# qyber-black/Code-RobChar

Hardware: AMD Instinct MI355X
Metric: MC fidelity evals/sec (N=7, 100 ctrls x 10k draws) (higher is better)
Workload: dtype f64

## Files before the change

### code-robchar_amd/csrc/k_fidelity_chain.inc.h

```cpp
constexpr int kWavesSmall = 5;
constexpr int fid_min_waves(int n, int mode) {
    if (mode == rc::kWeightsAdjugate)
        return n >= 17 ? 1
               : rc::kSumRuleMoments >= 3 ? (n <= 6 ? kWavesSmall : (n <= 7 ? 4 : (n <= 8 ? 3 : (n >= 13 ? 1 : 2))))
                                          : (n <= 6 ? kWavesSmall : (n <= 8 ? 4 : (n == 13 ? 1 : 2)));
    if (mode == rc::kWeightsRows) return n <= 8 ? kWavesSmall : (n <= 12 ? 3 : 2);
    return n <= 6 ? kWavesSmall : (n <= 8 ? 4 : (n <= 10 ? 3 : (n <= 14 ? 2 : 1)));
}
constexpr int fid_phases(int n, int mode) { return n <= 2 ? 1 : (n <= 8 ? 2 : 4); }

#include "philox_core.inc.h"

__device__ unsigned long long g_general_tiles = 0;
__device__ unsigned long long g_polish_tiles[64] = {0};

struct LdsVec {
    double* base;
    int stride;
    __device__ __forceinline__ double& operator[](int i) const { return base[i * stride]; }
};

template <int N, int MODE>
__global__ __launch_bounds__(64, fid_min_waves(N, MODE)) void mc_fid_chain_kernel(const FidParams p) {
    constexpr int G = 3 * N;
    constexpr int PH = fid_phases(N, MODE);
    constexpr int SP = 64 / PH;
    constexpr int kPhaseBytes = SP * G * 8;
    __shared__ __attribute__((aligned(16))) double stage[SP * G];
    __shared__ __attribute__((aligned(16))) double sctab[128];

    const int lane = threadIdx.x;
    const long long tile = blockIdx.x;
    const double2 ent = reinterpret_cast<const double2*>(g_sincos_table)[lane];
    reinterpret_cast<double2*>(sctab)[lane] = ent;
    __builtin_amdgcn_s_setprio(3);
#ifdef RC_STAMPS
    const long long t_begin = __builtin_amdgcn_s_memtime();
    const long long r_begin = __builtin_amdgcn_s_memrealtime();
#endif
    const long long c = tile / p.tiles_per_ctrl;
    const long long kb = (tile - c * p.tiles_per_ctrl) * 64;
    const int nk = (int)((p.K - kb < 64) ? (p.K - kb) : 64);

    const double* xg = p.ctrl + c * (N + 1);
    double x[N + 1];
    bool pad = false;
#pragma unroll
    for (int i = 0; i <= N; ++i) {
        x[i] = xg[i];
        pad |= (x[i] != x[i]);
    }
#ifdef RC_STAMPS
    long long t_ph[4] = {0, 0, 0, 0};
    asm volatile("s_waitcnt lgkmcnt(0)" ::: "memory");
    const long long t_ctrl = __builtin_amdgcn_s_memtime();
#endif
    double* dst = p.fid + c * p.K + kb;
    if (pad) {
        if (lane < nk) dst[lane] = __builtin_nan("");
        return;
    }

    const char* src = (const char*)(p.draws + c * p.draw_cstride + kb * G);
    double gl[G];
#pragma unroll
    for (int ph = 0; ph < PH; ++ph) {
        const int first = ph * SP;
        if (first < nk) {
            const int cnt = (nk - first < SP) ? (nk - first) : SP;
            const int bytes = cnt * G * 8;
            const char* ps = src + (long long)first * G * 8;
            if (p.align16 && !(cnt & 1)) {
#pragma unroll
                for (int it = 0; it < (kPhaseBytes + 1023) / 1024; ++it) {
                    const int off = it * 1024 + lane * 16;
                    if (off < bytes)
                        __builtin_amdgcn_global_load_lds((rc_gptr_t)(ps + off),
                                                         (rc_lptr_t)((char*)stage + it * 1024), 16, 0, rckp::kDrawLoadAux);
                }
            } else {
#pragma unroll 2
                for (int it = 0; it < (kPhaseBytes + 255) / 256; ++it) {
                    const int off = it * 256 + lane * 4;
                    if (off < bytes)
                        __builtin_amdgcn_global_load_lds((rc_gptr_t)(ps + off),
                                                         (rc_lptr_t)((char*)stage + it * 256), 4, 0, rckp::kDrawLoadAux);
                }
            }
            asm volatile("s_waitcnt vmcnt(0)" ::: "memory");
#ifdef RC_STAMPS
            if (ph < 2) t_ph[2 * ph] = __builtin_amdgcn_s_memtime();
#endif
            int rel = lane - first;
            asm volatile("" : "+v"(rel));
            if (rel >= 0 && rel < cnt) {
#pragma unroll
                for (int i = 0; i < G; ++i) gl[i] = stage[rel * G + i];
            }
            asm volatile("s_waitcnt lgkmcnt(0)" ::: "memory");
#ifdef RC_STAMPS
            if (ph < 2) t_ph[2 * ph + 1] = __builtin_amdgcn_s_memtime();
#endif
        }
    }
    __builtin_amdgcn_s_setprio(0);
    __syncthreads();
#ifdef RC_STAMPS
    const long long t_loaded = __builtin_amdgcn_s_memtime();
#endif

    double f = 0.0;
    bool ok = true;
#ifdef RC_STAMPS
    long long t_in[2] = {0, 0};
    if (lane < nk)
        ok = rc::chain_fidelity_fast<N, MODE>(x, p.h0.diag, p.h0.off, [&gl](int i) { return gl[i]; }, p.in, p.out, sctab, f, t_in);
#else
    int extra = 0;
    if (lane < nk)
        ok = rc::chain_fidelity_fast<N, MODE>(x, p.h0.diag, p.h0.off, [&gl](int i) { return gl[i]; }, p.in, p.out, sctab, f,
                                              nullptr, &extra);
    if (extra && lane == 0) atomicAdd(&g_polish_tiles[blockIdx.x & 63u], 1ull);
#endif
    constexpr bool kRepairInRegisters = MODE != rc::kWeightsRows && N <= RC_MAX_NSPIN_FAST;
    unsigned long long badmask = __ballot(lane < nk && !ok);
    if (badmask != 0ull) {
        if (lane == 0) atomicAdd(&g_general_tiles, 1ull);
        if (kRepairInRegisters) {
            const bool bad = (badmask >> lane) & 1ull;
            bool ok2 = true;
            if (bad) {
                const double* gsrc = (const double*)src + (long long)lane * G;
                double f2;
                ok2 = rc::chain_fidelity_fast<N, rc::kWeightsRows>(xg, p.h0.diag, p.h0.off, [gsrc](int i) { return gsrc[i]; },
                                                                   p.in, p.out, sctab, f2);
                if (ok2) f = f2;
            }
            badmask = __ballot(bad && !ok2);
        }
    }
    if (badmask != 0ull) {
        constexpr int CH = (SP * G) / (4 * N);
        const bool bad = (badmask >> lane) & 1ull;
        const int rank = __popcll(badmask & ((1ull << lane) - 1ull));
        const int nbad = __popcll(badmask);
#pragma unroll 1
        for (int c0 = 0; c0 < nbad; c0 += CH) {
            const int rel = rank - c0;
            if (bad && rel >= 0 && rel < CH) {
                const LdsVec vd{stage + rel, CH}, ve{stage + N * CH + rel, CH}, va{stage + 2 * N * CH + rel, CH},
                    vb{stage + 3 * N * CH + rel, CH};
                f = rc::chain_fidelity_general(N, xg, p.h0.diag, p.h0.off,
                                               (const double*)src + (long long)lane * G, p.in, p.out, vd, ve, va, vb);
            }
        }
    }
    if (lane < nk) {
        if (p.nt_store) {
            __attribute__((address_space(1))) double* nt_dst = (__attribute__((address_space(1))) double*)(dst + lane);
            asm volatile("" : "+v"(nt_dst));
            __builtin_nontemporal_store(f, nt_dst);
        } else {
            dst[lane] = f;
        }
    }

#ifdef RC_STAMPS
    __builtin_amdgcn_s_waitcnt(0);
    const long long t_end = __builtin_amdgcn_s_memtime();
    if (lane == 0 && p.stamps) {
        long long* rec = p.stamps + tile * rckp::kStampSlots;
        rec[0] = t_begin;
        rec[1] = t_loaded;
        rec[2] = t_end;
        rec[3] = __builtin_amdgcn_s_memrealtime() - r_begin;
        rec[4] = t_ctrl;
        rec[5] = t_ph[0];
        rec[6] = t_in[0];
        rec[7] = t_in[1];
        rec[8] = (long long)__builtin_amdgcn_s_getreg(4 | (0 << 6) | (31 << 11));
        rec[9] = (long long)__builtin_amdgcn_s_getreg(20 | (0 << 6) | (31 << 11));
        rec[10] = r_begin;
        rec[11] = r_begin + rec[3];
    }
#endif
}

constexpr int kRingMaxN = 16;
constexpr int ring_min_waves(int n) { return n <= 4 ? 5 : (n <= 5 ? 4 : (n <= 6 ? 3 : (n <= 8 ? 2 : 1))); }


template <int N>
__device__ __forceinline__ void ring_tile_fp64(const FidParams& p, const double corner, const long long tile, double* stage,
                                               const double* sctab) {
    constexpr int G = 3 * N;
    constexpr int PH = fid_phases(N, rc::kWeightsRows);
    constexpr int SP = 64 / PH;
    const int lane = threadIdx.x;
    __builtin_amdgcn_s_setprio(3);
    const long long c = tile / p.tiles_per_ctrl;
    const long long kb = (tile - c * p.tiles_per_ctrl) * 64;
    const int nk = (int)((p.K - kb < 64) ? (p.K - kb) : 64);
    const double* xg = p.ctrl + c * (N + 1);
    double x[N + 1];
    bool pad = false;
#pragma unroll
    for (int i = 0; i <= N; ++i) {
        x[i] = xg[i];
        pad |= (x[i] != x[i]);
    }
    double* dst = p.fid + c * p.K + kb;
    if (pad) {
        if (lane < nk) dst[lane] = __builtin_nan("");
        __builtin_amdgcn_s_setprio(0);
        return;
    }
    const char* src = (const char*)(p.draws + c * p.draw_cstride + kb * G);
    double gl[G];
    stage_tile_draws<G, PH>(src, nk, lane, p.align16, stage, gl);
    __builtin_amdgcn_s_setprio(0);

    double f = 0.0;
    bool ok = true;
    if (lane < nk)
        ok = rc::ring_fidelity_fast<N>(x, p.h0.diag, p.h0.off, corner, [&gl](int i) { return gl[i]; }, p.in, p.out, sctab, f);
    const unsigned long long badmask = __ballot(lane < nk && !ok);
    if (badmask) {
        if (lane == 0) atomicAdd(&g_general_tiles, 1ull);
        constexpr int CH = (SP * G) / (6 * N);
        const bool bad = (badmask >> lane) & 1ull;
        const int rank = __popcll(badmask & ((1ull << lane) - 1ull));
        const int nbad = __popcll(badmask);
#pragma unroll 1
        for (int c0 = 0; c0 < nbad; c0 += CH) {
            const int rel = rank - c0;
            if (bad && rel >= 0 && rel < CH) {
                const LdsVec vd{stage + rel, CH}, ve{stage + N * CH + rel, CH};
                LdsVec vz[4] = {{stage + 2 * N * CH + rel, CH}, {stage + 3 * N * CH + rel, CH}, {stage + 4 * N * CH + rel, CH},
                                {stage + 5 * N * CH + rel, CH}};
                const double* gsrc = (const double*)src + (long long)lane * G;
                f = rc::ring_fidelity_general<N>(x, p.h0.diag, p.h0.off, corner, [gsrc](int i) { return gsrc[i]; }, p.in, p.out,
                                                 vd, ve, vz);
            }
        }
    }
    if (lane < nk) dst[lane] = f;
}

template <int N>
__global__ __launch_bounds__(64, ring_min_waves(N)) void mc_fid_ring_kernel(const FidParams p, const double corner) {
    constexpr int G = 3 * N;
    constexpr int SP = 64 / fid_phases(N, rc::kWeightsRows);
    __shared__ __attribute__((aligned(16))) double stage[SP * G];
    __shared__ __attribute__((aligned(16))) double sctab[128];
    const double2 ent = reinterpret_cast<const double2*>(g_sincos_table)[threadIdx.x];
    reinterpret_cast<double2*>(sctab)[threadIdx.x] = ent;
    __syncthreads();
    ring_tile_fp64<N>(p, corner, blockIdx.x, stage, sctab);
}

constexpr int ring_mixed_min_waves(int n) {
    return n <= 4 ? 5 : (n <= 6 ? 4 : (n <= 8 ? 3 : (n == 9 ? (rc::kSumRuleMoments >= 3 ? 2 : 3) : (n <= 13 ? 2 : 1))));
}


template <int N>
__global__ __launch_bounds__(64, ring_mixed_min_waves(N)) void mc_fid_ring_mixed_kernel(const FidParams p, const double corner,
                                                                                        const RingRepairList rl) {
    constexpr int G = 3 * N;
    constexpr int PH = (N == 16) ? 8 : fid_phases(N, rc::kWeightsEnds);
    constexpr int SP = 64 / PH;
    __shared__ __attribute__((aligned(16))) double stage[SP * G];
    __shared__ __attribute__((aligned(16))) double sctab[128];
    const int lane = threadIdx.x;
    const long long tile = blockIdx.x;
    if (blockIdx.x == 0 && lane == 0) *rl.clear = 0ull;
    const double2 ent = reinterpret_cast<const double2*>(g_sincos_table)[lane];
    reinterpret_cast<double2*>(sctab)[lane] = ent;
    __builtin_amdgcn_s_setprio(3);
    const long long c = tile / p.tiles_per_ctrl;
    const long long kb = (tile - c * p.tiles_per_ctrl) * 64;
    const int nk = (int)((p.K - kb < 64) ? (p.K - kb) : 64);
    const double* xg = p.ctrl + c * (N + 1);
    double x[N + 1];
    bool pad = false;
#pragma unroll
    for (int i = 0; i <= N; ++i) {
        x[i] = xg[i];
        pad |= (x[i] != x[i]);
    }
    double* dst = p.fid + c * p.K + kb;
    if (pad) {
        if (lane < nk) dst[lane] = __builtin_nan("");
        return;
    }
    const char* src = (const char*)(p.draws + c * p.draw_cstride + kb * G);
    double gl[G];
    stage_tile_draws<G, PH>(src, nk, lane, p.align16, stage, gl);
    __builtin_amdgcn_s_setprio(0);
    __syncthreads();
    double f = 0.0;
    bool ok = true;
    int extra = 0;
    if (lane < nk)
        ok = rc::ring_fidelity_mixed<N>(x, p.h0.diag, p.h0.off, corner, [&gl](int i) { return gl[i]; }, p.in, p.out, sctab, f,
                                        &extra);
    if (extra && lane == 0) atomicAdd(&g_polish_tiles[blockIdx.x & 63u], 1ull);
    const bool bad = lane < nk && !ok;
    const unsigned long long badmask = __ballot(bad);
    if (badmask) {
        const int first = __ffsll((long long)badmask) - 1;
        unsigned long long base = 0;
        if (lane == first) base = atomicAdd(rl.count, (unsigned long long)__popcll(badmask));
        base = __shfl(base, first, 64);
        if (bad) {
            rl.samples[base + __popcll(badmask & ((1ull << lane) - 1ull))] = c * p.K + kb + lane;
            f = __builtin_nan("");
        }
    }
    if (lane < nk) dst[lane] = f;
}

template <int N>
__global__ __launch_bounds__(64, 1) void mc_fid_ring_repair_kernel(const FidParams p, const double corner, const RingRepairList rl) {
    constexpr int G = 3 * N;
    __shared__ __attribute__((aligned(16))) double work[6 * N * 64];
    __shared__ __attribute__((aligned(16))) double sctab[128];
    const int lane = threadIdx.x;
    const double2 ent = reinterpret_cast<const double2*>(g_sincos_table)[lane];
    reinterpret_cast<double2*>(sctab)[lane] = ent;
// ... 62 lines not shown
```

### code-robchar_amd/csrc/robchar_hip.hip

```cpp
#include <hip/hip_runtime.h>

#include <dlfcn.h>
#include <math.h>
#include <stdint.h>
#include <stdlib.h>
#include <string.h>
#include <atomic>
#include <initializer_list>
#include <mutex>
#include <unordered_map>
#include <thread>
#include <string>
#include <vector>

#include "../../include/robchar_hip.h"
#include "kernel_params.h"
#include "tridiag_core.h"
#include "hermitian_core.h"
#include "csym_core.h"
#include "sort_core.h"
#include "select_core.h"
#include "bootstrap_core.h"
#include "wasserstein_core.h"
#include "lbfgs_core.h"
// ... 57 lines not shown
std::mutex g_cfg_mu;
int g_default_kernel = RC_KERNEL_AUTO;
long long* g_stamps = nullptr;

constexpr int kMaxDevices = 64;
enum { kAttrExpm = 0, kAttrAnyN, kAttrSortMerge, kAttrSortChunk, kAttrMtJump, kAttrMtJumpWide, kAttrCount };
struct RingBuf {
    char* mem = nullptr;
    long long cap = 0;
    int turn = 0;
    unsigned long long last_use = 0;
};
constexpr size_t kMaxRingBufs = 16;
struct DeviceCtx {
    std::mutex mu;
    hipStream_t stream = nullptr;
    void* ws = nullptr;
    size_t ws_bytes = 0;
    std::mutex ring_mu;
    std::unordered_map<hipStream_t, RingBuf> ring_bufs;
    unsigned long long ring_clock = 0;
    std::atomic<bool> attr[kAttrCount];
    DeviceCtx() {
        for (auto& a : attr) a.store(false);
    }
};
DeviceCtx g_ctx[kMaxDevices];

int device_in_range(int device) {
    int n = 0;
    RC_HIP_CHECK(hipGetDeviceCount(&n));
    if (device < 0 || device >= n || device >= kMaxDevices) return fail(RC_EINVAL, "device index out of range");
    return RC_OK;
}

int get_ctx(int device, DeviceCtx** out) {
    if (int rc = device_in_range(device)) return rc;
    RC_HIP_CHECK(hipSetDevice(device));
    if (!g_ctx[device].stream) RC_HIP_CHECK(hipStreamCreateWithFlags(&g_ctx[device].stream, hipStreamNonBlocking));
    *out = &g_ctx[device];
    return RC_OK;
}

int ensure_func_attr(int which, const void* func, int bytes) {
    int dev = 0;
    RC_HIP_CHECK(hipGetDevice(&dev));
    if (dev < 0 || dev >= kMaxDevices) return fail(RC_EINVAL, "device index out of range");
    if (g_ctx[dev].attr[which].load(std::memory_order_acquire)) return RC_OK;
    RC_HIP_CHECK(hipFuncSetAttribute(func, hipFuncAttributeMaxDynamicSharedMemorySize, bytes));
    g_ctx[dev].attr[which].store(true, std::memory_order_release);
    return RC_OK;
}

int ensure_ws(DeviceCtx* ctx, size_t bytes) {
    if (ctx->ws_bytes >= bytes) return RC_OK;
    if (ctx->ws) RC_HIP_CHECK(hipFree(ctx->ws));
    ctx->ws = nullptr;
    ctx->ws_bytes = 0;
    RC_HIP_CHECK(hipMalloc(&ctx->ws, bytes));
    ctx->ws_bytes = bytes;
    return RC_OK;
}

bool is_device_ptr(const void* p) {
    hipPointerAttribute_t attr;
    hipError_t e = hipPointerGetAttributes(&attr, p);
    if (e != hipSuccess) {
        (void)hipGetLastError();
        return false;
    }
    return attr.type == hipMemoryTypeDevice;
}

struct Staging {
    DeviceCtx* ctx = nullptr;
    rcws::Plan plan;
    int in(const void* p, size_t bytes) { return plan.in(p, bytes, is_device_ptr(p)); }
    int out(void* p, size_t bytes, bool always = false) { return plan.out(p, bytes, p && !always && is_device_ptr(p), always); }
    double* ptr(int slot) const { return (double*)plan.ptr(slot, ctx->ws); }
    int stage_in() {
        if (int rc = ensure_ws(ctx, plan.total)) return rc;
        for (int i = 0; i < plan.n; ++i)
            if (const rcws::Slot& s = plan.s[i]; s.input && s.staged)
                RC_HIP_CHECK(hipMemcpyAsync(ptr(i), s.user, s.bytes, hipMemcpyHostToDevice, ctx->stream));
        return RC_OK;
    }
    int stage_out() {
        for (int i = 0; i < plan.n; ++i)
            if (const rcws::Slot& s = plan.s[i]; !s.input && s.staged && s.user)
                RC_HIP_CHECK(hipMemcpyAsync((void*)s.user, ptr(i), s.bytes, s.always ? hipMemcpyDefault : hipMemcpyDeviceToHost,
                                            ctx->stream));
        RC_HIP_CHECK(hipStreamSynchronize(ctx->stream));
        return RC_OK;
    }
};

struct StreamFree {
    void* p;
    hipStream_t s;
    ~StreamFree() {
        if (p) (void)hipFreeAsync(p, s);
    }
};

void fill_h0(StaticH& h0, int N, const double* h0_diag, const double* h0_offdiag) {
    for (int i = 0; i < RC_MAX_NSPIN; ++i) {
        h0.diag[i] = (h0_diag && i < N) ? h0_diag[i] : 0.0;
        h0.off[i] = (i < N - 1) ? (h0_offdiag ? h0_offdiag[i] : 1.0) : 0.0;
    }
}

int check_common(int N, int in, int out, long long C, long long K) {
    if (N < 2 || N > RC_MAX_NSPIN) return fail(RC_EINVAL, "N must be in [2, 32]");
    if (in < 0 || in >= N || out < 0 || out >= N) return fail(RC_EINVAL, "in/out spin index out of range");
    if (C < 0 || K < 0) return fail(RC_EINVAL, "C and K must be non-negative");
    return RC_OK;
}

int ring_buf_reserve(RingBuf& rb, hipStream_t s, long long samples) {
    if (rb.cap >= samples && rb.mem) return RC_OK;
    if (rb.mem) RC_HIP_CHECK(hipFreeAsync(rb.mem, s));
    rb.mem = nullptr;
    rb.cap = 0;
    const long long cap = samples + (samples >> 2);
    RC_HIP_CHECK(hipMallocAsync((void**)&rb.mem, 256 + (size_t)cap * sizeof(long long), s));
    RC_HIP_CHECK(hipMemsetAsync(rb.mem, 0, 256, s));
    rb.cap = cap;
    rb.turn = 0;
    return RC_OK;
}

RingBuf& ring_buf_for(DeviceCtx& ctx, hipStream_t s) {
    auto it = ctx.ring_bufs.find(s);
    if (it == ctx.ring_bufs.end()) {
        if (ctx.ring_bufs.size() >= kMaxRingBufs) {
            auto old = ctx.ring_bufs.begin();
            for (auto j = ctx.ring_bufs.begin(); j != ctx.ring_bufs.end(); ++j)
                if (j->second.last_use < old->second.last_use) old = j;
            if (old->second.mem) (void)hipFree(old->second.mem);
            ctx.ring_bufs.erase(old);
        }
        it = ctx.ring_bufs.emplace(s, RingBuf{}).first;
    }
    it->second.last_use = ++ctx.ring_clock;
    return it->second;
}

constexpr long long kNtStoreTiles = 32768;
std::atomic<long long> g_nt_store_tiles{kNtStoreTiles};

template <int N, int MODE>
int launch_chain(hipStream_t s, const FidParams& p0, long long nt_store_tiles) {
    const long long blocks = p0.ntiles;
    if (blocks > 0x7fffffffLL) return fail(RC_EINVAL, "too many tiles for one launch");
    FidParams p = p0;
    p.nt_store = (blocks < nt_store_tiles) ? 1 : 0;
    hipLaunchKernelGGL((mc_fid_chain_kernel<N, MODE>), dim3((unsigned)blocks), dim3(64), 0, s, p);
    RC_HIP_CHECK(hipGetLastError());
    return RC_OK;
}

int enqueue_expm(hipStream_t s, int N, int in, int out, const double* h0_diag, const double* h0_offdiag, int ring,
                 const double* ctrl, const double* draws, long long draw_cstride, const double* diag_imag,
                 long long imag_cstride, long long C, long long K, double* fid, bool fast_complex_diagonal = false) {
    if (N > RC_MAX_NSPIN_FAST) return fail(RC_EINVAL, "the dense kernels (ring topology, expm) support N <= 16");
    ExpmParams p{};
    p.ctrl = ctrl;
    p.draws = draws;
    p.diag_imag = diag_imag;
    p.fid = fid;
    p.C = C;
    p.K = K;
    p.draw_cstride = draw_cstride;
    p.imag_cstride = imag_cstride;
    p.N = N;
    p.in = in;
    p.out = out;
    p.ring = ring ? 1 : 0;
    fill_h0(p.h0, N, h0_diag, h0_offdiag);
    const size_t lds = (size_t)kExpmWaves * kExpmBufs * N * N * sizeof(cplx);
    if (int rc = ensure_func_attr(kAttrExpm, (const void*)mc_fid_expm_kernel,
                                  kExpmWaves * kExpmBufs * RC_MAX_NSPIN_FAST * RC_MAX_NSPIN_FAST * (int)sizeof(cplx)))
        return rc;
    const long long total = C * K;
    long long blocks = (total + kExpmWaves - 1) / kExpmWaves;
    if (blocks > 256LL * 16) blocks = 256LL * 16;
    if (fast_complex_diagonal && !ring && N <= kCsymMaxN) {
        const long long cblocks = (total + 63) / 64;
        if (cblocks > 0x7fffffffLL) return fail(RC_EINVAL, "too many samples for one launch");
        switch (N) {
#define RC_CSYM_CASE(n) \
    case n: hipLaunchKernelGGL(mc_fid_csym_kernel<n>, dim3((unsigned)cblocks), dim3(64), 0, s, p); break;
            RC_CSYM_CASE(2) RC_CSYM_CASE(3) RC_CSYM_CASE(4) RC_CSYM_CASE(5) RC_CSYM_CASE(6) RC_CSYM_CASE(7) RC_CSYM_CASE(8)
            RC_CSYM_CASE(9) RC_CSYM_CASE(10) RC_CSYM_CASE(11) RC_CSYM_CASE(12)
#undef RC_CSYM_CASE
        }
        p.only_marked = 1;
    }
    hipLaunchKernelGGL(mc_fid_expm_kernel, dim3((unsigned)blocks), dim3(64 * kExpmWaves), lds, s, p);
    RC_HIP_CHECK(hipGetLastError());
    return RC_OK;
}

int draws_align16(const double* draws, long long draw_cstride) {
    return (((uintptr_t)draws & 15) == 0 && (((size_t)draw_cstride * 8) & 15) == 0) ? 1 : 0;
}
size_t draws_bytes(long long C, long long K, int N, long long stride) {
    return (stride == 0 ? (size_t)K * N * 3 : ((size_t)(C - 1) * stride + (size_t)K * N * 3)) * sizeof(double);
}

int enqueue_fidelity(hipStream_t s, int kernel, int N, int in, int out, const double* h0_diag,
                     const double* h0_offdiag, int ring, const double* ctrl, const double* draws,
                     long long draw_cstride, long long C, long long K, double* fid) {
    if (draw_cstride < 0) draw_cstride = K * N * 3;
    if (draw_cstride != 0 && draw_cstride < K * N * 3) return fail(RC_EINVAL, "draws_ctrl_stride overlaps controllers");
    if (int rc = check_common(N, in, out, C, K)) return rc;
    if (C == 0 || K == 0) return RC_OK;
    if (!ctrl || !draws || !fid) return fail(RC_EINVAL, "NULL array pointer");
    const bool ends = (in == 0 && out == N - 1) || (in == N - 1 && out == 0);
    if (ring && N == 2) ring = 0;
    const bool mixed_ring = (kernel == RC_KERNEL_AUTO) && ring && N <= kRingMaxN;
    if (kernel == RC_KERNEL_AUTO)
        kernel = ring ? (N <= kRingMaxN ? RC_KERNEL_RING_HH : RC_KERNEL_JACOBI) : RC_KERNEL_TRIDIAG_ADJ;
    if (kernel == RC_KERNEL_RING_HH) {
        if (!ring) return fail(RC_EINVAL, "RC_KERNEL_RING_HH is the ring-topology kernel (chains: the tridiagonal kernels)");
        if (N > kRingMaxN) return fail(RC_EINVAL, "the lane-per-sample ring kernels support N <= 16");
        FidParams p{};
        p.ctrl = ctrl;
        p.draws = draws;
        p.fid = fid;
        p.C = C;
        p.K = K;
        p.draw_cstride = draw_cstride;
        p.tiles_per_ctrl = (K + 63) / 64;
        p.ntiles = C * p.tiles_per_ctrl;
        p.in = in;
        p.out = out;
        p.align16 = draws_align16(draws, draw_cstride);
        fill_h0(p.h0, N, h0_diag, h0_offdiag);
        if (p.ntiles > 0x7fffffffLL) return fail(RC_EINVAL, "too many tiles for one launch");
        const dim3 grid((unsigned)p.ntiles);
        if (mixed_ring) {
            RingRepairList rl{};
            {
                int dev = 0;
                RC_HIP_CHECK(hipGetDevice(&dev));
                if (dev < 0 || dev >= kMaxDevices) return fail(RC_EINVAL, "device index out of range");
                std::lock_guard<std::mutex> lk(g_ctx[dev].ring_mu);
                RingBuf& rb = ring_buf_for(g_ctx[dev], s);
                if (int rc = ring_buf_reserve(rb, s, C * K)) return rc;
                rl.count = (unsigned long long*)(rb.mem + 64 * rb.turn);
                rl.clear = (unsigned long long*)(rb.mem + 64 * (rb.turn ^ 1));
                rl.samples = (long long*)(rb.mem + 256);
                rb.turn ^= 1;
            }
            static const long long kRepairGrid = [] {
                const char* e = getenv("RC_RING_REPAIR_GRID");
                const long long v = e ? atoll(e) : 0;
                return v > 0 ? v : 1024LL;
            }();
            const long long nwaves = (C * K + 63) / 64;
            const dim3 rgrid((unsigned)(nwaves < kRepairGrid ? nwaves : kRepairGrid));
            if (N > 10) {
                RC_HIP_CHECK((hipError_t)rc_large_ring_launch(N, 1, (void*)s, &p, 1.0, &rl, grid.x, rgrid.x));
                return RC_OK;
            }
            switch (N) {
#define RC_RING_CASE(n)                                                                         \
    case n:                                                                                     \
        hipLaunchKernelGGL(mc_fid_ring_mixed_kernel<n>, grid, dim3(64), 0, s, p, 1.0, rl);      \
        hipLaunchKernelGGL(mc_fid_ring_repair_kernel<n>, rgrid, dim3(64), 0, s, p, 1.0, rl);    \
        break;
                RC_RING_CASE(3) RC_RING_CASE(4) RC_RING_CASE(5) RC_RING_CASE(6) RC_RING_CASE(7) RC_RING_CASE(8) RC_RING_CASE(9)
                RC_RING_CASE(10)
#undef RC_RING_CASE
            }
            RC_HIP_CHECK(hipGetLastError());
            return RC_OK;
        }
        if (N > 10) {
            RC_HIP_CHECK((hipError_t)rc_large_ring_launch(N, 0, (void*)s, &p, 1.0, nullptr, grid.x, 0u));
            return RC_OK;
        }
        switch (N) {
#define RC_RING_CASE(n) \
    case n: hipLaunchKernelGGL(mc_fid_ring_kernel<n>, grid, dim3(64), 0, s, p, 1.0); break;
            RC_RING_CASE(3) RC_RING_CASE(4) RC_RING_CASE(5) RC_RING_CASE(6) RC_RING_CASE(7) RC_RING_CASE(8) RC_RING_CASE(9)
            RC_RING_CASE(10)
#undef RC_RING_CASE
        }
        RC_HIP_CHECK(hipGetLastError());
        return RC_OK;
    }
    if (kernel == RC_KERNEL_TRIDIAG_QL || kernel == RC_KERNEL_TRIDIAG_ADJ) {
        const int mode = (kernel == RC_KERNEL_TRIDIAG_QL) ? rc::kWeightsRows
                                                          : ((ends && N <= 14) ? rc::kWeightsEnds : rc::kWeightsAdjugate);
        if (ring) return fail(RC_EINVAL, "the tridiagonal QL kernel handles chain topology only");
        FidParams p{};
        p.ctrl = ctrl;
        p.draws = draws;
        p.fid = fid;
        p.C = C;
        p.K = K;
        p.draw_cstride = draw_cstride;
        p.tiles_per_ctrl = (K + 63) / 64;
        p.ntiles = C * p.tiles_per_ctrl;
        p.in = in;
        p.out = out;
        p.align16 = draws_align16(draws, draw_cstride);
        p.stamps = g_stamps;
        fill_h0(p.h0, N, h0_diag, h0_offdiag);
        if (N > RC_MAX_NSPIN_CHAIN || (N > RC_MAX_NSPIN_FAST && mode == rc::kWeightsRows)) {
            const long long blocks = p.ntiles;
            if (blocks > 0x7fffffffLL) return fail(RC_EINVAL, "too many tiles for one launch");
            const size_t lds = (size_t)4 * N * 64 * sizeof(double);
            if (int rc = ensure_func_attr(kAttrAnyN, (const void*)mc_fid_chain_anyn_kernel, 4 * RC_MAX_NSPIN * 64 * (int)sizeof(double)))
                return rc;
            hipLaunchKernelGGL(mc_fid_chain_anyn_kernel, dim3((unsigned)blocks), dim3(64), lds, s, p, N);
            RC_HIP_CHECK(hipGetLastError());
            return RC_OK;
        }
        if (N > RC_MAX_NSPIN_FAST) {
            if (p.ntiles > 0x7fffffffLL) return fail(RC_EINVAL, "too many tiles for one launch");
            RC_HIP_CHECK((hipError_t)rc_large_chain_launch(N, (void*)s, &p));
            return RC_OK;
        }
        const long long nt_tiles = g_nt_store_tiles.load(std::memory_order_relaxed);
        switch (N) {
#define RC_CASE(n)                                                                        \
    case n:                                                                               \
        return mode == rc::kWeightsRows ? launch_chain<n, rc::kWeightsRows>(s, p, nt_tiles)         \
               : (mode == rc::kWeightsEnds ? launch_chain<n, rc::kWeightsEnds>(s, p, nt_tiles)      \
                                           : launch_chain<n, rc::kWeightsAdjugate>(s, p, nt_tiles));
#define RC_CASE_ADJ_ROWS(n)                                                               \
    case n:                                                                               \
        return mode == rc::kWeightsRows ? launch_chain<n, rc::kWeightsRows>(s, p, nt_tiles) : launch_chain<n, rc::kWeightsAdjugate>(s, p, nt_tiles);
#ifdef RC_DEV_FEW_N
            RC_CASE(5) RC_CASE(7) RC_CASE(10)
#else
            RC_CASE(2) RC_CASE(3) RC_CASE(4) RC_CASE(5) RC_CASE(6) RC_CASE(7) RC_CASE(8) RC_CASE(9)
            RC_CASE(10) RC_CASE(11) RC_CASE(12) RC_CASE(13) RC_CASE(14) RC_CASE_ADJ_ROWS(15) RC_CASE_ADJ_ROWS(16)
#endif
#undef RC_CASE
#undef RC_CASE_ADJ_ROWS
        }
        return fail(RC_EINVAL, "unsupported N");
    }
    if (N > RC_MAX_NSPIN_FAST) return fail(RC_EINVAL, "the dense kernels (ring topology, expm) support N <= 16");
    if (kernel == RC_KERNEL_EXPM)
        return enqueue_expm(s, N, in, out, h0_diag, h0_offdiag, ring, ctrl, draws, draw_cstride, nullptr, 0, C, K, fid);
    if (kernel == RC_KERNEL_JACOBI) {
        JacParams p{};
        p.ctrl = ctrl;
        p.draws = draws;
        p.fid = fid;
        p.C = C;
        p.K = K;
        p.draw_cstride = draw_cstride;
        p.N = N;
        p.in = in;
        p.out = out;
        p.ring = ring ? 1 : 0;
        fill_h0(p.h0, N, h0_diag, h0_offdiag);
        const long long total = C * K;
        const int spw = (N <= 8) ? 8 : 4;
        long long blocks = (total + kJacWaves * spw - 1) / (kJacWaves * spw);
        if (blocks > 256LL * 16) blocks = 256LL * 16;
        if (N <= 8)
            hipLaunchKernelGGL((mc_fid_jacobi_kernel<8, 8>), dim3((unsigned)blocks), dim3(64 * kJacWaves), 0, s, p);
        else
            hipLaunchKernelGGL((mc_fid_jacobi_kernel<16, 16>), dim3((unsigned)blocks), dim3(64 * kJacWaves), 0, s, p);
        RC_HIP_CHECK(hipGetLastError());
        return RC_OK;
    }
    return fail(RC_EINVAL, "unknown kernel id");
}

int enqueue_reduce(hipStream_t s, const double* fid, long long C, long long K, const double* thr, int nq,
                   double eps, double* rim1, double* stdv, double* minf, double* q, double* sorted_out, bool standalone = false) {
    if (C < 0 || K < 0) return fail(RC_EINVAL, "C and K must be non-negative");
    if (nq < 0 || nq > kMaxQ) return fail(RC_EINVAL, "nq must be in [0, 8]");
    if (nq > 0 && !thr) return fail(RC_EINVAL, "q_thresholds is NULL");
    if (C == 0) return RC_OK;
    if (K == 0) return fail(RC_EINVAL, "K must be positive for a reduction");
    if (!fid) return fail(RC_EINVAL, "NULL fid pointer");
    if (C > 0x7fffffffLL) return fail(RC_EINVAL, "too many controllers for one launch");
    RedParams p{};
    p.fid = fid;
    p.C = C;
    p.K = K;
    p.nq = nq;
    for (int j = 0; j < nq; ++j) p.thr[j] = thr[j];
    p.eps = eps;
    p.rim1 = rim1;
    p.stdv = stdv;
    p.minf = minf;
    p.q = q;
    if (rim1 || stdv || minf || q) {
        if (K <= kWaveRowMaxK && C >= 64) {
            const dim3 grid((unsigned)((C + 3) / 4));
            if (nq == 0)
                hipLaunchKernelGGL(reduce_rows_wave_kernel<0>, grid, dim3(256), 0, s, p);
            else if (nq <= 2)
                hipLaunchKernelGGL(reduce_rows_wave_kernel<2>, grid, dim3(256), 0, s, p);
            else
                hipLaunchKernelGGL(reduce_rows_wave_kernel<kMaxQ>, grid, dim3(256), 0, s, p);
        } else if (nq <= 2 && K > kWaveRowMaxK && K <= 32LL * 128) {
            if (nq == 0) hipLaunchKernelGGL((reduce_kernel<0, 128>), dim3((unsigned)C), dim3(128), 0, s, p);
            else hipLaunchKernelGGL((reduce_kernel<2, 128>), dim3((unsigned)C), dim3(128), 0, s, p);
        } else if (nq <= 2 && K > kWaveRowMaxK && K <= 32LL * 256) {
            if (nq == 0) hipLaunchKernelGGL((reduce_kernel<0, 256>), dim3((unsigned)C), dim3(256), 0, s, p);
            else hipLaunchKernelGGL((reduce_kernel<2, 256>), dim3((unsigned)C), dim3(256), 0, s, p);
        } else if (standalone && nq <= 2 && K > 32LL * 256 && K <= 40LL * 256) {
            if (nq == 0) hipLaunchKernelGGL((reduce_kernel<0, 256, 40>), dim3((unsigned)C), dim3(256), 0, s, p);
            else hipLaunchKernelGGL((reduce_kernel<2, 256, 40>), dim3((unsigned)C), dim3(256), 0, s, p);
        } else if (nq == 0)
            hipLaunchKernelGGL(reduce_kernel<0>, dim3((unsigned)C), dim3(kRedThreads), 0, s, p);
        else if (nq <= 2)
            hipLaunchKernelGGL(reduce_kernel<2>, dim3((unsigned)C), dim3(kRedThreads), 0, s, p);
        else
            hipLaunchKernelGGL(reduce_kernel<kMaxQ>, dim3((unsigned)C), dim3(kRedThreads), 0, s, p);
        RC_HIP_CHECK(hipGetLastError());
    }
    if (sorted_out) {
        long long P = 2;
        while (P < K) P <<= 1;
        if (C * P > (1LL << 34)) return fail(RC_EINVAL, "sorted_out: workspace would exceed 128 GiB");
        if (K <= kSortChunk) {
            if (int rc = ensure_func_attr(kAttrSortMerge, (const void*)sort_rows_merge_kernel, (kSortChunk / 16 * 17 + 1) * 8))
                return rc;
            const int T = (int)((K + 15) / 16), n = 16 * T;
            const int threads = ((T + 63) / 64) * 64;
            hipLaunchKernelGGL(sort_rows_merge_kernel, dim3((unsigned)C), dim3(threads), (size_t)(n / 16 * 17 + 1) * sizeof(double),
                               s, fid, sorted_out, K, n);
            RC_HIP_CHECK(hipGetLastError());
            return RC_OK;
        }
        struct SortWs {
            double* work = nullptr;
            int* flags = nullptr;
        } wsv, *ws = &wsv;
        RC_HIP_CHECK(hipMallocAsync((void**)&wsv.work, (size_t)C * P * sizeof(double), s));
        if (hipError_t e = hipMallocAsync((void**)&wsv.flags, (size_t)C * sizeof(int), s); e != hipSuccess) {
            (void)hipFreeAsync(wsv.work, s);
            return fail(RC_EHIP, std::string("hipMallocAsync(sort flags): ") + hipGetErrorString(e));
        }
        struct Release {
            SortWs* w;
            hipStream_t st;
            ~Release() {
                (void)hipFreeAsync(w->work, st);
                (void)hipFreeAsync(w->flags, st);
            }
        } release{ws, s};
        RC_HIP_CHECK(hipMemsetAsync(ws->flags, 0, (size_t)C * sizeof(int), s));
        {
            if (int rc = ensure_func_attr(kAttrSortChunk, (const void*)sort_chunk16_kernel, kSortChunk / 16 * 17 * 8)) return rc;
            const size_t lds16 = (size_t)(kSortChunk / 16 * 17) * sizeof(double);
            const dim3 cgrid((unsigned)C, (unsigned)(P / kSortChunk));
            hipLaunchKernelGGL(sort_chunk16_kernel, cgrid, dim3(kSortThreads), lds16, s, fid, ws->work, sorted_out, ws->flags,
                               K, P, 2LL, (long long)kSortChunk, 1, 0);
            for (long long size = 2LL * kSortChunk; size <= P; size <<= 1) {
                long long hi = size >> 1;
                while (hi >= kSortChunk) {
                    int nleft = 0;
                    for (long long x = hi; x >= kSortChunk; x >>= 1) ++nleft;
                    const int take = nleft >= 4 ? 4 : nleft;
                    const long long S = hi >> (take - 1);
                    const dim3 ggrid((unsigned)C, 128);
                    switch (take) {
                        case 4: hipLaunchKernelGGL(sort_global_fused_kernel<4>, ggrid, dim3(256), 0, s, ws->work, P, size, S); break;
                        case 3: hipLaunchKernelGGL(sort_global_fused_kernel<3>, ggrid, dim3(256), 0, s, ws->work, P, size, S); break;
                        case 2: hipLaunchKernelGGL(sort_global_fused_kernel<2>, ggrid, dim3(256), 0, s, ws->work, P, size, S); break;
                        default: hipLaunchKernelGGL(sort_global_fused_kernel<1>, ggrid, dim3(256), 0, s, ws->work, P, size, S); break;
                    }
                    hi = S >> 1;
// ... 1892 lines not shown
```

### code-robchar_amd/csrc/robchar_large.hip

```cpp
#include <hip/hip_runtime.h>

#include <math.h>
#include <stdint.h>

#include "../../include/robchar_hip.h"
#include "kernel_params.h"
#include "tridiag_core.h"
#include "hermitian_core.h"

namespace {

using rckp::StaticH;
using rckp::FidParams;
using rckp::RingRepairList;
#include "tile_stage.inc.h"

#include "k_fidelity_chain.inc.h"

}

extern "C" {

__attribute__((visibility("hidden"))) int rc_large_chain_launch(int N, void* stream, const rckp::FidParams* pp) {
    const FidParams& p = *pp;
    hipStream_t s = (hipStream_t)stream;
    const dim3 grid((unsigned)p.ntiles);
    switch (N) {
#define RC_CASE_ADJ(n) \
    case n: hipLaunchKernelGGL((mc_fid_chain_kernel<n, rc::kWeightsAdjugate>), grid, dim3(64), 0, s, p); break;
#ifndef RC_DEV_FEW_N
        RC_CASE_ADJ(17) RC_CASE_ADJ(18) RC_CASE_ADJ(19) RC_CASE_ADJ(20) RC_CASE_ADJ(21) RC_CASE_ADJ(22) RC_CASE_ADJ(23) RC_CASE_ADJ(24)
#endif
#undef RC_CASE_ADJ
        default: return (int)hipErrorInvalidValue;
    }
    return (int)hipGetLastError();
}

__attribute__((visibility("hidden"))) int rc_large_ring_launch(int N, int mixed, void* stream, const rckp::FidParams* pp, double corner,
                                                               const rckp::RingRepairList* rlp, unsigned grid, unsigned rgrid) {
    const FidParams& p = *pp;
    hipStream_t s = (hipStream_t)stream;
    switch (N) {
#define RC_RING_CASE(n)                                                                                         \
    case n:                                                                                                     \
        if (mixed) {                                                                                            \
            hipLaunchKernelGGL(mc_fid_ring_mixed_kernel<n>, dim3(grid), dim3(64), 0, s, p, corner, *rlp);       \
            hipLaunchKernelGGL(mc_fid_ring_repair_kernel<n>, dim3(rgrid), dim3(64), 0, s, p, corner, *rlp);     \
        } else {                                                                                                \
            hipLaunchKernelGGL(mc_fid_ring_kernel<n>, dim3(grid), dim3(64), 0, s, p, corner);                   \
        }                                                                                                       \
        break;
#ifndef RC_DEV_FEW_N
        RC_RING_CASE(11) RC_RING_CASE(12) RC_RING_CASE(13) RC_RING_CASE(14) RC_RING_CASE(15) RC_RING_CASE(16)
#endif
#undef RC_RING_CASE
        default: return (int)hipErrorInvalidValue;
    }
    return (int)hipGetLastError();
}

__attribute__((visibility("hidden"))) int rc_large_counter_addr(int which, void** addr) {
    return which == 0 ? (int)hipGetSymbolAddress(addr, HIP_SYMBOL(g_general_tiles))
                      : (int)hipGetSymbolAddress(addr, HIP_SYMBOL(g_polish_tiles));
}

}
```

### code-robchar_amd/csrc/tile_stage.inc.h

```cpp
#pragma once

typedef __attribute__((address_space(1))) const void* rc_gptr_t;
typedef __attribute__((address_space(3))) void* rc_lptr_t;

template <int G, int PH, int AUX = rckp::kDrawLoadAux>
__device__ __forceinline__ void stage_tile_draws(const char* src, int nk, int lane, int align16, double* stage, double (&gl)[G]) {
    constexpr int SP = 64 / PH;
    constexpr int kPhaseBytes = SP * G * 8;
#pragma unroll
    for (int ph = 0; ph < PH; ++ph) {
        const int first = ph * SP;
        if (first < nk) {
            const int cnt = (nk - first < SP) ? (nk - first) : SP;
            const int bytes = cnt * G * 8;
            const char* ps = src + (long long)first * G * 8;
            if (align16 && !(cnt & 1)) {
#pragma unroll
                for (int it = 0; it < (kPhaseBytes + 1023) / 1024; ++it) {
                    const int off = it * 1024 + lane * 16;
                    if (off < bytes)
                        __builtin_amdgcn_global_load_lds((rc_gptr_t)(ps + off), (rc_lptr_t)((char*)stage + it * 1024), 16, 0, AUX);
                }
            } else {
#pragma unroll 2
                for (int it = 0; it < (kPhaseBytes + 255) / 256; ++it) {
                    const int off = it * 256 + lane * 4;
                    if (off < bytes)
                        __builtin_amdgcn_global_load_lds((rc_gptr_t)(ps + off), (rc_lptr_t)((char*)stage + it * 256), 4, 0, AUX);
                }
            }
            asm volatile("s_waitcnt vmcnt(0)" ::: "memory");
            int rel = lane - first;
            asm volatile("" : "+v"(rel));
            if (rel >= 0 && rel < cnt) {
#pragma unroll
                for (int i = 0; i < G; ++i) gl[i] = stage[rel * G + i];
            }
            asm volatile("s_waitcnt lgkmcnt(0)" ::: "memory");
        }
    }
}
```

Before: 19.27 billion.

## Double-buffer draw staging into sub-phases and use a 3D grid to drop tile division

Splits each staging phase into two smaller sub-phases and double-buffers them in LDS, so the DMA of the next sub-phase overlaps the register readout of the current one under partial vmcnt waits. A fully aligned full-tile path uses compile-time unrolled 16-byte DMA with immediate offsets. The ctrl-row load and NaN check are moved after the first DMA issues, and the sincos table write is moved after staging. The launch becomes a 3D grid (tile, ctrl, ctrl-chunk), which removes the 64-bit division per block. This adds code complexity and relies on vmcnt counts matching the issued loads exactly.

```diff
diff --git a/code-robchar_amd/csrc/k_fidelity_chain.inc.h b/code-robchar_amd/csrc/k_fidelity_chain.inc.h
--- a/code-robchar_amd/csrc/k_fidelity_chain.inc.h
+++ b/code-robchar_amd/csrc/k_fidelity_chain.inc.h
@@ -20,89 +20,159 @@
     __device__ __forceinline__ double& operator[](int i) const { return base[i * stride]; }
 };
 
+constexpr unsigned kCtrlPerGridZ = 32768;
+inline bool chain_grid_fits(const FidParams& p) { return p.ntiles <= 0x7fffffffLL && p.C <= 65535LL * kCtrlPerGridZ; }
+inline dim3 chain_grid(const FidParams& p) {
+    return dim3((unsigned)p.tiles_per_ctrl, (unsigned)(p.C < kCtrlPerGridZ ? p.C : kCtrlPerGridZ),
+                (unsigned)((p.C + kCtrlPerGridZ - 1) / kCtrlPerGridZ));
+}
 template <int N, int MODE>
 __global__ __launch_bounds__(64, fid_min_waves(N, MODE)) void mc_fid_chain_kernel(const FidParams p) {
     constexpr int G = 3 * N;
     constexpr int PH = fid_phases(N, MODE);
     constexpr int SP = 64 / PH;
-    constexpr int kPhaseBytes = SP * G * 8;
-    __shared__ __attribute__((aligned(16))) double stage[SP * G];
-    __shared__ __attribute__((aligned(16))) double sctab[128];
+    constexpr int NS = (PH == 1) ? 1 : 2 * PH;
+    constexpr int SS = 64 / NS;
+    constexpr int kSubBytes = SS * G * 8;
+    constexpr int kDma16 = (kSubBytes + 1023) / 1024, kDma4 = (kSubBytes + 255) / 256;
+    static_assert(kSubBytes % 16 == 0 && kDma4 <= 31 && (NS == 1 || 2 * SS * G == SP * G), "staging geometry");
+    __shared__ __attribute__((aligned(16))) double lds[SP * G + 128];
+    double* const stage = lds;
+    double* const sctab = lds + SP * G;
 
     const int lane = threadIdx.x;
-    const long long tile = blockIdx.x;
     const double2 ent = reinterpret_cast<const double2*>(g_sincos_table)[lane];
-    reinterpret_cast<double2*>(sctab)[lane] = ent;
-    __builtin_amdgcn_s_setprio(3);
 #ifdef RC_STAMPS
     const long long t_begin = __builtin_amdgcn_s_memtime();
     const long long r_begin = __builtin_amdgcn_s_memrealtime();
 #endif
-    const long long c = tile / p.tiles_per_ctrl;
-    const long long kb = (tile - c * p.tiles_per_ctrl) * 64;
+    const unsigned cu = blockIdx.z * kCtrlPerGridZ + blockIdx.y, kt = blockIdx.x;
+    if (blockIdx.z != 0 && cu >= (unsigned long long)p.C) return;
+    const long long c = cu;
+    const long long kb = (long long)kt * 64;
     const int nk = (int)((p.K - kb < 64) ? (p.K - kb) : 64);
+    int align16 = p.align16;
+    asm("" : "+s"(align16));
 
     const double* xg = p.ctrl + c * (N + 1);
     double x[N + 1];
-    bool pad = false;
-#pragma unroll
-    for (int i = 0; i <= N; ++i) {
-        x[i] = xg[i];
-        pad |= (x[i] != x[i]);
-    }
-#ifdef RC_STAMPS
-    long long t_ph[4] = {0, 0, 0, 0};
-    asm volatile("s_waitcnt lgkmcnt(0)" ::: "memory");
-    const long long t_ctrl = __builtin_amdgcn_s_memtime();
-#endif
+#pragma unroll
+    for (int i = 0; i <= N; ++i) x[i] = xg[i];
+    __builtin_amdgcn_s_setprio(3);
+
     double* dst = p.fid + c * p.K + kb;
-    if (pad) {
-        if (lane < nk) dst[lane] = __builtin_nan("");
-        return;
-    }
 
     const char* src = (const char*)(p.draws + c * p.draw_cstride + kb * G);
-    double gl[G];
-#pragma unroll
-    for (int ph = 0; ph < PH; ++ph) {
-        const int first = ph * SP;
-        if (first < nk) {
-            const int cnt = (nk - first < SP) ? (nk - first) : SP;
+    const bool full = (nk == 64) && align16;
+    auto issue = [&](auto full_c, const int s) __attribute__((always_inline)) {
+        const int first = s * SS;
+        char* half = (char*)stage + (s & 1) * kSubBytes;
+        if constexpr (decltype(full_c)::value) {
+            dma16_pieces<kSubBytes, rckp::kDrawLoadAux>(src + (long long)s * kSubBytes + lane * 16, half, lane * 16);
+        } else if (first < nk) {
+            const int cnt = (nk - first < SS) ? (nk - first) : SS;
             const int bytes = cnt * G * 8;
             const char* ps = src + (long long)first * G * 8;
-            if (p.align16 && !(cnt & 1)) {
-#pragma unroll
-                for (int it = 0; it < (kPhaseBytes + 1023) / 1024; ++it) {
+            if (align16 && !(cnt & 1)) {
+#pragma unroll
+                for (int it = 0; it < kDma16; ++it) {
                     const int off = it * 1024 + lane * 16;
                     if (off < bytes)
-                        __builtin_amdgcn_global_load_lds((rc_gptr_t)(ps + off),
-                                                         (rc_lptr_t)((char*)stage + it * 1024), 16, 0, rckp::kDrawLoadAux);
+                        __builtin_amdgcn_global_load_lds((rc_gptr_t)(ps + off), (rc_lptr_t)(half + it * 1024), 16, 0,
+                                                         rckp::kDrawLoadAux);
                 }
             } else {
 #pragma unroll 2
-                for (int it = 0; it < (kPhaseBytes + 255) / 256; ++it) {
+                for (int it = 0; it < kDma4; ++it) {
                     const int off = it * 256 + lane * 4;
                     if (off < bytes)
-                        __builtin_amdgcn_global_load_lds((rc_gptr_t)(ps + off),
-                                                         (rc_lptr_t)((char*)stage + it * 256), 4, 0, rckp::kDrawLoadAux);
+                        __builtin_amdgcn_global_load_lds((rc_gptr_t)(ps + off), (rc_lptr_t)(half + it * 256), 4, 0,
+                                                         rckp::kDrawLoadAux);
                 }
             }
-            asm volatile("s_waitcnt vmcnt(0)" ::: "memory");
-#ifdef RC_STAMPS
-            if (ph < 2) t_ph[2 * ph] = __builtin_amdgcn_s_memtime();
-#endif
-            int rel = lane - first;
-            asm volatile("" : "+v"(rel));
-            if (rel >= 0 && rel < cnt) {
-#pragma unroll
-                for (int i = 0; i < G; ++i) gl[i] = stage[rel * G + i];
+        }
+    };
+    constexpr rc_bool_c<true> kFullPath{};
+    constexpr rc_bool_c<false> kGeneralPath{};
+    if (full) {
+        issue(kFullPath, 0);
+        if (NS > 1) issue(kFullPath, 1);
+    } else {
+        issue(kGeneralPath, 0);
+        if (NS > 1) issue(kGeneralPath, 1);
+    }
+
+    bool pad = false;
+#pragma unroll
+    for (int i = 0; i <= N; ++i) pad |= (x[i] != x[i]);
+#ifdef RC_STAMPS
+    long long t_ph0 = 0;
+    asm volatile("s_waitcnt lgkmcnt(0)" ::: "memory");
+    const long long t_ctrl = __builtin_amdgcn_s_memtime();
+#endif
+    if (pad) {
+        asm volatile("s_waitcnt vmcnt(0)" ::: "memory");
+        if (lane < nk) dst[lane] = __builtin_nan("");
+        return;
+    }
+
+    if constexpr (MODE == rc::kWeightsRows) {
+#pragma unroll
+        for (int i = 0; i <= N; ++i) asm("" : "+v"(x[i]));
+    }
+    double gl[G];
+#ifdef RC_STAMPS
+#define RC_STAMP_PH0(s) if ((s) == 0) t_ph0 = __builtin_amdgcn_s_memtime()
+#else
+#define RC_STAMP_PH0(s) (void)0
+#endif
+    if (full) {
+        int mine[2] = {(lane % SS) * G, (lane % SS) * G + SS * G};
+        asm("" : "+v"(mine[0]));
+        asm("" : "+v"(mine[1]));
+#pragma unroll
+        for (int s = 0; s < NS; ++s) {
+            if (s + 1 < NS)
+                asm volatile("s_waitcnt vmcnt(%0)" ::"n"(kDma16) : "memory");
+            else
+                asm volatile("s_waitcnt vmcnt(0)" ::: "memory");
+            RC_STAMP_PH0(s);
+            if (lane / SS == s) {
+#pragma unroll
+                for (int i = 0; i < G; ++i) gl[i] = stage[mine[s & 1] + i];
             }
             asm volatile("s_waitcnt lgkmcnt(0)" ::: "memory");
-#ifdef RC_STAMPS
-            if (ph < 2) t_ph[2 * ph + 1] = __builtin_amdgcn_s_memtime();
-#endif
-        }
-    }
+            if (s + 2 < NS) issue(kFullPath, s + 2);
+        }
+    } else {
+#pragma unroll
+        for (int s = 0; s < NS; ++s) {
+            const int first = s * SS;
+            if (first < nk) {
+                const int cnt = (nk - first < SS) ? (nk - first) : SS;
+                if (s + 1 < NS && first + 2 * SS <= nk) {
+                    if (align16)
+                        asm volatile("s_waitcnt vmcnt(%0)" ::"n"(kDma16) : "memory");
+                    else
+                        asm volatile("s_waitcnt vmcnt(%0)" ::"n"(kDma4) : "memory");
+                } else {
+                    asm volatile("s_waitcnt vmcnt(0)" ::: "memory");
+                }
+                RC_STAMP_PH0(s);
+                const int rel = lane - first;
+                int at = rel * G + (s & 1) * (SS * G);
+                asm volatile("" : "+v"(at));
+                if (rel >= 0 && rel < cnt) {
+#pragma unroll
+                    for (int i = 0; i < G; ++i) gl[i] = stage[at + i];
+                }
+                asm volatile("s_waitcnt lgkmcnt(0)" ::: "memory");
+                if (s + 2 < NS) issue(kGeneralPath, s + 2);
+            }
+        }
+    }
+#undef RC_STAMP_PH0
+    reinterpret_cast<double2*>(sctab)[lane] = ent;
     __builtin_amdgcn_s_setprio(0);
     __syncthreads();
 #ifdef RC_STAMPS
@@ -120,7 +190,7 @@
     if (lane < nk)
         ok = rc::chain_fidelity_fast<N, MODE>(x, p.h0.diag, p.h0.off, [&gl](int i) { return gl[i]; }, p.in, p.out, sctab, f,
                                               nullptr, &extra);
-    if (extra && lane == 0) atomicAdd(&g_polish_tiles[blockIdx.x & 63u], 1ull);
+    if (extra && lane == 0) atomicAdd(&g_polish_tiles[(kt + cu) & 63u], 1ull);
 #endif
     constexpr bool kRepairInRegisters = MODE != rc::kWeightsRows && N <= RC_MAX_NSPIN_FAST;
     unsigned long long badmask = __ballot(lane < nk && !ok);
@@ -169,13 +239,13 @@
     __builtin_amdgcn_s_waitcnt(0);
     const long long t_end = __builtin_amdgcn_s_memtime();
     if (lane == 0 && p.stamps) {
-        long long* rec = p.stamps + tile * rckp::kStampSlots;
+        long long* rec = p.stamps + (c * p.tiles_per_ctrl + kt) * rckp::kStampSlots;
         rec[0] = t_begin;
         rec[1] = t_loaded;
         rec[2] = t_end;
         rec[3] = __builtin_amdgcn_s_memrealtime() - r_begin;
         rec[4] = t_ctrl;
-        rec[5] = t_ph[0];
+        rec[5] = t_ph0;
         rec[6] = t_in[0];
         rec[7] = t_in[1];
         rec[8] = (long long)__builtin_amdgcn_s_getreg(4 | (0 << 6) | (31 << 11));
diff --git a/code-robchar_amd/csrc/robchar_hip.hip b/code-robchar_amd/csrc/robchar_hip.hip
--- a/code-robchar_amd/csrc/robchar_hip.hip
+++ b/code-robchar_amd/csrc/robchar_hip.hip
@@ -233,10 +233,10 @@
 template <int N, int MODE>
 int launch_chain(hipStream_t s, const FidParams& p0, long long nt_store_tiles) {
     const long long blocks = p0.ntiles;
-    if (blocks > 0x7fffffffLL) return fail(RC_EINVAL, "too many tiles for one launch");
+    if (!chain_grid_fits(p0)) return fail(RC_EINVAL, "too many tiles for one launch");
     FidParams p = p0;
     p.nt_store = (blocks < nt_store_tiles) ? 1 : 0;
-    hipLaunchKernelGGL((mc_fid_chain_kernel<N, MODE>), dim3((unsigned)blocks), dim3(64), 0, s, p);
+    hipLaunchKernelGGL((mc_fid_chain_kernel<N, MODE>), chain_grid(p), dim3(64), 0, s, p);
     RC_HIP_CHECK(hipGetLastError());
     return RC_OK;
 }
@@ -402,7 +402,7 @@
             return RC_OK;
         }
         if (N > RC_MAX_NSPIN_FAST) {
-            if (p.ntiles > 0x7fffffffLL) return fail(RC_EINVAL, "too many tiles for one launch");
+            if (!chain_grid_fits(p)) return fail(RC_EINVAL, "too many tiles for one launch");
             RC_HIP_CHECK((hipError_t)rc_large_chain_launch(N, (void*)s, &p));
             return RC_OK;
         }
diff --git a/code-robchar_amd/csrc/robchar_large.hip b/code-robchar_amd/csrc/robchar_large.hip
--- a/code-robchar_amd/csrc/robchar_large.hip
+++ b/code-robchar_amd/csrc/robchar_large.hip
@@ -24,7 +24,7 @@
 __attribute__((visibility("hidden"))) int rc_large_chain_launch(int N, void* stream, const rckp::FidParams* pp) {
     const FidParams& p = *pp;
     hipStream_t s = (hipStream_t)stream;
-    const dim3 grid((unsigned)p.ntiles);
+    const dim3 grid = chain_grid(p);
     switch (N) {
 #define RC_CASE_ADJ(n) \
     case n: hipLaunchKernelGGL((mc_fid_chain_kernel<n, rc::kWeightsAdjugate>), grid, dim3(64), 0, s, p); break;
diff --git a/code-robchar_amd/csrc/tile_stage.inc.h b/code-robchar_amd/csrc/tile_stage.inc.h
--- a/code-robchar_amd/csrc/tile_stage.inc.h
+++ b/code-robchar_amd/csrc/tile_stage.inc.h
@@ -2,6 +2,25 @@
 
 typedef __attribute__((address_space(1))) const void* rc_gptr_t;
 typedef __attribute__((address_space(3))) void* rc_lptr_t;
+
+template <bool B>
+struct rc_bool_c {
+    static constexpr bool value = B;
+};
+
+template <int BYTES, int AUX, int IT = 0>
+__device__ __forceinline__ void dma16_pieces(const char* gsrc_lane, char* lds, int lane16) {
+    static_assert(BYTES % 16 == 0, "16-byte pieces");
+    if constexpr (IT * 1024 < BYTES) {
+        constexpr int off = IT * 1024, hi = off & ~4095, lo = off & 4095;
+        if constexpr (off + 1024 <= BYTES) {
+            __builtin_amdgcn_global_load_lds((rc_gptr_t)(gsrc_lane + hi), (rc_lptr_t)(lds + hi), 16, lo, AUX);
+        } else {
+            if (lane16 < BYTES - off) __builtin_amdgcn_global_load_lds((rc_gptr_t)(gsrc_lane + hi), (rc_lptr_t)(lds + hi), 16, lo, AUX);
+        }
+        dma16_pieces<BYTES, AUX, IT + 1>(gsrc_lane, lds, lane16);
+    }
+}
 
 template <int G, int PH, int AUX = rckp::kDrawLoadAux>
 __device__ __forceinline__ void stage_tile_draws(const char* src, int nk, int lane, int align16, double* stage, double (&gl)[G]) {
```

New measurement: 19.48 billion (median of 6 runs). +1.1%, better.
